# anrieff/fray

Measured on AMD Instinct MI355X. Metric: Mrays/s (closest-hit + shadow rays) at 1920x1080, 64spp path trace, higher is better.
Workload: dtype f64

## Files before the change

fray_amd/csrc/adaptive_variant.hip:

```cpp
#include "adaptive.hpp"
#include "dev_compact.hpp"
#include "render_impl.hpp"

#ifndef FRAY_ST
#error "compile with -DFRAY_ST=0..5, 8 or 9"
#endif

namespace {

struct ListBatch {
    const int* list;
    int p0, np, s0, cn;
};

static __global__ __launch_bounds__(256) void k_seed_list(DFrame F, ListBatch B, uint32_t* __restrict__ x397)
{
    constexpr int NC = FRAY_SEED_CHAINS;
    const uint32_t total = (uint32_t)B.np * (uint32_t)B.cn;
    const uint32_t groups = (total + NC - 1u) / NC;
    for (uint32_t q = blockIdx.x * blockDim.x + threadIdx.x; q < groups; q += gridDim.x * blockDim.x) {
        uint32_t b[NC], slot[NC];
#pragma unroll
        for (int k = 0; k < NC; k++) {
            slot[k] = q + (uint32_t)k * groups;
// ... 25 lines not shown
        const int i = (int)(slot % (uint32_t)B.np), s = (int)(slot / (uint32_t)B.np);
        int x, y;
        item_pixel(F, B.list[B.p0 + i], x, y);
        PathState ps;
        const uint32_t p = (uint32_t)y * (uint32_t)F.W + (uint32_t)x;
        ps.rnd = mt_seed_with(sample_seed(F.seed, p, (uint32_t)(B.s0 + s)), x397[slot]);
        ps.tab = ps.rnd;
        float ox = rng_float(ps.rnd), oy = rng_float(ps.rnd);
        double fx = (double)((float)x + ox), fy = (double)((float)y + oy);
        if (C.dof) dof_ray(C, fx, fy, ps.tab, ps.o, ps.d); else screen_ray(C, fx, fy, ps.o, ps.d);
        ps.pm = c3(1, 1, 1);
        ps.slot = slot;
        ps.depth = 0;
        ps.flags = 0;
        c.samples++;
        path_store<FRAY_SORT && sort_variant(ST)>(Q, slot, ps, ray_sort_class<ST>(ps.d, 0u));
        termCount[slot] = 0;
    }
    if (ST & 1) flush_stats(st, c);
    else if (c.samples) atomicAdd(&st->samples, c.samples);
}

struct PixelState {
    float* sum;
    float* prev;
    unsigned char* flag;
};

struct ResolveArgs {
    DFrame F;
    ListBatch B;
// ... 218 lines not shown
```

fray_amd/csrc/capi.hip:

```cpp
#include <hip/hip_runtime.h>

#include <algorithm>
#include <chrono>
#include <cstddef>
#include <cmath>
#include <cstring>
#include <string>
#include <vector>
#include <functional>
#include <cstdlib>


#include "entry_support.hpp"
#include "dev_rng.hpp"
#include "dev_pack.hpp"
#include "scene_arena.hpp"

namespace {

using frayhip_detail::set_error;

void put3(double* o, const double* p) { o[0] = p[0]; o[1] = p[1]; o[2] = p[2]; }
}

// ... 215 lines not shown
    if (s->settings.gi) spp = std::max(spp, s->settings.numPaths);
    return spp;
}

DScene frame_scene(const frayhip_scene* s)
{
    const frayhip_settings& set = s->settings;
    DScene S = s->S;
    S.ambient[0] = set.ambientLight[0]; S.ambient[1] = set.ambientLight[1]; S.ambient[2] = set.ambientLight[2];
    S.maxTraceDepth = set.maxTraceDepth;
    S.gi = set.gi;
    S.saturation = set.saturation;
    S.skipNullSegments = s->skipNullSegments ? 1 : 0;
    S.segmentPlanes = s->segmentPlanes ? 1 : 0;
    S.certifiedSegments = (s->certifiedSegments && s->segmentPlanes && S.segCertAll) ? 1 : 0;
    if (!s->cameraSkip) S.nCamSkip = 0;
    if (!s->shadeShortcuts) S.shadeIdentity = S.lightsDiagonal = S.subdShift = 0;
    return S;
}

DFrame frame_record(const frayhip_scene* s, int bucketFirst, int bucketStride, uint32_t seed)
{
    DFrame F = frame_grid(s->settings.frameWidth, s->settings.frameHeight);
    F.bucketStride = bucketStride > 0 ? bucketStride : 1;
    F.bucketFirst = bucketFirst;
    F.nBuckets = frayhip_bucket_count(F.W, F.H, F.bucketFirst, F.bucketStride);
    F.spp = frame_spp(s);
    F.seed = seed;
    F.jitter = (s->camera.dof || s->settings.gi) ? 1 : 0;
    return F;
// ... 305 lines not shown
    sc->edit = make_scene_edit(d, B);
    sc->camera = d.camera;
    sc->settings = d.settings;
    if (hipMalloc((void**)&sc->d_stats, kStatsBytes) != hipSuccess || hipMalloc((void**)&sc->d_qmeta, 3 * FRAY_PT_LANES * sizeof(QMeta)) != hipSuccess ||
        hipEventCreate(&sc->evA) != hipSuccess || hipEventCreate(&sc->evB) != hipSuccess || !create_lanes(sc)) {
        set_error("frayhip_scene_create: could not allocate the per-scene device state");
        frayhip_scene_destroy(sc);
        return FRAYHIP_E_NOMEM;
    }
    if (const char* e = getenv("FRAYHIP_PT_LANES")) { long v = atol(e); if (v >= 1 && v <= FRAY_PT_LANES) sc->ptLanes = (int)v; }
    if (const char* e = getenv("FRAYHIP_SPECULATE_FANS")) sc->speculateFans = atol(e) != 0;
    if (const char* e = getenv("FRAYHIP_FP_CONTRACT")) sc->fpContract = atol(e) == 1;
    if (const char* e = getenv("FRAYHIP_SKIP_NULL_SEGMENTS")) sc->skipNullSegments = atol(e) != 0;
    if (const char* e = getenv("FRAYHIP_SEGMENT_PLANES")) sc->segmentPlanes = atol(e) != 0;
    if (const char* e = getenv("FRAYHIP_CERTIFIED_SEGMENTS")) sc->certifiedSegments = atol(e) != 0;
    if (const char* e = getenv("FRAYHIP_TIGHT_GATES")) sc->tightGates = atol(e) != 0;
    if (const char* e = getenv("FRAYHIP_CAMERA_SKIP")) sc->cameraSkip = atol(e) != 0;
    if (const char* e = getenv("FRAYHIP_CAMERA_TILES")) sc->cameraTiles = atol(e) != 0;
    if (const char* e = getenv("FRAYHIP_SHADE_SHORTCUTS")) sc->shadeShortcuts = atol(e) != 0;
    if (const char* e = getenv("FRAYHIP_FUSED_WHITTED_MAX")) { long v = atol(e); if (v >= 0 && v <= 1024) sc->fusedWhittedMax = (int)v; }
    if (const char* e = getenv("FRAYHIP_CSG_LANES")) { long v = atol(e); if (v >= 1 && v <= FRAY_PT_LANES) sc->csgLanes = (int)v; }
    if (const char* e = getenv("FRAYHIP_SEED_TABLE_MIB")) { long v = atol(e); if (v >= 0 && v <= (1 << 20)) sc->seedTableCapBytes = (size_t)v << 20; }
    if (const char* e = getenv("FRAYHIP_PT_BUDGET_MIB")) { long v = atol(e); if (v >= 1 && v <= (1 << 20)) { sc->ptBudgetBytes = (size_t)v << 20; sc->ptBudgetEff = 0; } }
    *out = sc;
    return FRAYHIP_OK;
}

int frayhip_scene_get_option(frayhip_scene* s, const char* name, int64_t* value)
{
    if (!s || !name || !value) { set_error("frayhip_scene_get_option: null argument"); return FRAYHIP_E_ARG; }
// ... 355 lines not shown
```

fray_amd/csrc/dev_scene.hpp:

```cpp
#pragma once
#include <stdint.h>
#include "frayhip.h"
#include "dev_tricert.hpp"
#include "dev_segcert.hpp"
#include "dev_gatecert.hpp"

#ifdef __HIP_DEVICE_COMPILE__
#define FRAY_RO __attribute__((address_space(4)))
#else
#define FRAY_RO
#endif

#define FRAY_CSG_MAX 30
#ifndef FRAY_CSG_DEPTH
#define FRAY_CSG_DEPTH 16
#endif

#define FRAY_KD_LDS_STACK 16
#define FRAY_KD_MAX_DEPTH 72

struct DXform { double off[3]; double m[9]; double inv[9]; };

struct DTri;
struct DNode {
// ... 126 lines not shown
    const FRAY_RO DLight* lights;
    DEnv env;
    int32_t nNodes, nLights;
    float probPickLight;
    float ambient[3];
    int32_t maxTraceDepth, gi;
    float saturation;
    const FRAY_RO DSegPlane* segPlanes;
    const FRAY_RO uint32_t* segNodeMasks;
    int32_t nSegPlanes, nSegNodes;
    int32_t segmentPlanes;
    int32_t skipNullSegments;
    int32_t segCertAll;
    int32_t certifiedSegments;
    const FRAY_RO DCamSkip* camSkip;
    int32_t nCamSkip, padCamSkip;
    const FRAY_RO double* worldNormals;
    int32_t normStride, shadeIdentity, lightsDiagonal;
    int32_t subdShift;
};

struct DFrame {
    int32_t W, H, BW, BH;
    int32_t bucketFirst, bucketStride, nBuckets , spp;
    uint32_t seed;
    int32_t jitter;
};

struct DStats {
    unsigned long long closest, shadow, node, kdInner, leafRefs, tri, prim, smooth, samples, tex, rngOverflow;
#ifdef FRAY_STAMPS
// ... 6 lines not shown
```

fray_amd/csrc/kernels.hpp:

```cpp
#pragma once
#include "dev_shade.hpp"
#include "dev_whitted.hpp"
#include "dev_queues.hpp"
#include "dev_camtile.hpp"
#include <type_traits>

#ifndef FRAY_PRIMARY_WAVES
#define FRAY_PRIMARY_WAVES 5
#endif
#ifndef FRAY_WHITTED_WAVES
#define FRAY_WHITTED_WAVES 3
#endif
#ifndef FRAY_WHITTED_REFILL
#define FRAY_WHITTED_REFILL 64
#endif
#ifndef FRAY_CSG_WAVES
#define FRAY_CSG_WAVES 3
#endif
constexpr int waves_for(int st, int n) { return (st & 2) ? (FRAY_CSG_WAVES < n ? FRAY_CSG_WAVES : n) : ((st & 1) && n > 2 ? n - 1 : n); }
#ifndef FRAY_MT_EARLY
#define FRAY_MT_EARLY 160
#endif
#ifndef FRAY_WH_SHADE_WAVES
#define FRAY_WH_SHADE_WAVES 4
// ... 748 lines not shown

#ifndef FRAY_SORT
#define FRAY_SORT 1
#endif
#ifndef FRAY_SORT_N
#define FRAY_SORT_N 1024
#endif
#ifdef FRAY_SORT_BY_MATERIAL
constexpr bool sort_variant(int) { return true; }
#else
#ifndef FRAY_SORT_CSG
#define FRAY_SORT_CSG 0
#endif
constexpr bool sort_variant(int st) { return (st & 6) == 4 || (FRAY_SORT_CSG && (st & 2) != 0); }
#endif
FD void wave_lds_sync()
{
    __builtin_amdgcn_fence(__ATOMIC_RELEASE, "wavefront");
    __builtin_amdgcn_wave_barrier();
    __builtin_amdgcn_fence(__ATOMIC_ACQUIRE, "wavefront");
}
template <class KeyOf>
FD void sort_share(const FRAY_RO uint32_t* off, const FRAY_RO uint32_t* nf, uint32_t nSeg, uint32_t chunk, uint32_t b0, uint32_t b1, uint32_t& seg,
                   uint32_t* buf, uint32_t* cnt, KeyOf keyOf)
{
    const uint32_t lane = threadIdx.x & 63u;
    if (lane < 16) cnt[lane] = 0;
    wave_lds_sync();
    uint32_t s1 = seg;
    for (uint32_t base = b0; base < b1; base += 64u) {
        const uint32_t di = base + lane;
        const bool live = di < b1;
        const uint32_t i = seg_map(off, nf, nSeg, chunk, base, di, live, s1) & ~FRAY_FRONT_BIT;
        if (live) atomicAdd(cnt + keyOf(i), 1u);
    }
    wave_lds_sync();
    {
        const uint32_t v = lane < 16 ? cnt[lane] : 0u;
        uint32_t inc = v;
        for (int d = 1; d < 16; d <<= 1) { const uint32_t t = __shfl_up(inc, d, 64); if ((int)lane >= d) inc += t; }
        wave_lds_sync();
        if (lane < 16) cnt[lane] = inc - v;
    }
    wave_lds_sync();
    uint32_t s2 = seg;
    for (uint32_t base = b0; base < b1; base += 64u) {
        const uint32_t di = base + lane;
        const bool live = di < b1;
        const uint32_t raw = seg_map(off, nf, nSeg, chunk, base, di, live, s2);
        if (live) buf[atomicAdd(cnt + keyOf(raw & ~FRAY_FRONT_BIT), 1u)] = raw;
    }
    seg = s2;
    wave_lds_sync();
}

template <class G>
FD void path_finish(const TermBuf& TB, DStats* st, const PathStateT<G>& s, const StereoBuf& SB)
{
    const Mt &r = cursor(s.rnd), &t = cursor(s.tab);
    if (SB.g[0]) {
        SB.g[0][s.slot] = r.j; SB.g[1][s.slot] = r.a; SB.g[2][s.slot] = r.b;
        SB.g[3][s.slot] = t.j; SB.g[4][s.slot] = t.a; SB.g[5][s.slot] = t.b;
    }
    TB.n[s.slot] = (unsigned short)(TB.b + 1);
    if (sizeof(G) == sizeof(Mt) && (r.j > 227 || t.j > 227)) atomicAdd(&st->rngOverflow, 1ull);
}
FD void term_store(const TermBuf& TB, uint32_t slot, C3 v)
// ... 28 lines not shown
                    if (C.dof) dof_ray(C, fx, fy, ps.tab, ro, rd, 2); else screen_ray(C, fx, fy, ro, rd, 2);
                    SB.r[0][slot] = ro.x; SB.r[1][slot] = ro.y; SB.r[2][slot] = ro.z;
                    SB.r[3][slot] = rd.x; SB.r[4][slot] = rd.y; SB.r[5][slot] = rd.z;
                }
            } else {
                ps.rnd.j = SB.g[0][slot]; ps.rnd.a = SB.g[1][slot]; ps.rnd.b = SB.g[2][slot];
                ps.tab.j = SB.g[3][slot]; ps.tab.a = SB.g[4][slot]; ps.tab.b = SB.g[5][slot];
                ps.o = v3(SB.r[0][slot], SB.r[1][slot], SB.r[2][slot]);
                ps.d = v3(SB.r[3][slot], SB.r[4][slot], SB.r[5][slot]);
            }
            ps.pm = c3(1, 1, 1);
            ps.slot = slot;
            ps.depth = 0;
            ps.flags = 0;
            bump<ST>(c.samples);
            path_store<FRAY_SORT && sort_variant(ST)>(Q, slot, ps, ray_sort_class<ST>(ps.d, 0u));
        } else {
            PathRec* r = Q.rec + slot;
            r->d[0] = 0; r->d[1] = 0; r->d[2] = 0;
            r->depthFlags = FRAY_DEAD;
            if constexpr (FRAY_SORT && sort_variant(ST)) Q.cls[slot] = 15;
        }
        termCount[slot] = 0;
    }
    if (ST & 1) flush_stats(st, c);
}

struct WaveShare { uint32_t begin, end, chunk, w, W; };
FD WaveShare wave_share(uint32_t n)
{
    WaveShare r;
    r.W = gridDim.x * (blockDim.x >> 6);
    r.w = blockIdx.x * (blockDim.x >> 6) + (threadIdx.x >> 6);
    r.chunk = (((n + r.W - 1u) / r.W) + 63u) & ~63u;
    r.begin = r.w * r.chunk;
    r.end = r.begin + r.chunk < n ? r.begin + r.chunk : n;
// ... 49 lines not shown
                if constexpr (ST == 0 && FRAY_ARITH == 0) { if (S.certifiedSegments) planesPass = segment_certified(S, sa, sb); }
                shadowBack = ray_gate_class<tight_variant(ST)>(S, sa, sb - sa);
                if constexpr (ST == 0) {
                    if (FRAY_ARITH == 0 ? planesPass && shadowBack == 0 : segment_surely_visible(S, sa, sb, shadowBack)) {
                        own = sc;
                        shadow = false;
                        atomicAdd(shadowEnds.n + 2, 1u);
                    }
                }
                if (ST != 0 || shadow) {
                    const uint32_t j = seg_take(shadowEnds, shadowBack != 0);
                    SQ.ax[j] = sa.x; SQ.ay[j] = sa.y; SQ.az[j] = sa.z;
                    SQ.bx[j] = sb.x; SQ.by[j] = sb.y; SQ.bz[j] = sb.z;
                    SQ.cr[j] = sc.r; SQ.cg[j] = sc.g; SQ.cb[j] = sc.b;
                    SQ.slot[j] = ps.slot;
                    if constexpr (FRAY_SORT && sort_variant(ST)) SQ.cls[j] = (unsigned char)ray_sort_class<ST>(sb - sa, shadowBack);
                }
            }
        }
        PathRay win, wout;
        win.o = ps.o; win.d = ps.d; win.depth = ps.depth; win.flags = ps.flags;
        C3 brdf;
        float pdf;
        spawn_ray(sh, info, win, ps.tab, wout, brdf, pdf);
        {
            ps.pm = ps.pm * brdf / pdf;
            ps.o = wout.o; ps.d = wout.d; ps.depth = wout.depth; ps.flags = wout.flags;
#ifdef FRAY_SORT_BY_MATERIAL
            ps.flags = (ps.flags & 0xffu) | ((sh.kind == 1 ? 0u : sh.kind == 3 ? 1u : sh.kind == 4 ? 2u : 3u) << 8);
#endif
            if (ps.depth > S.maxTraceDepth || intensity(ps.pm) < 0.01) path_finish(TB, st, ps, SB);
// ... 20 lines not shown
        const CamTileRays R = cam_tile_rays(V, x0, y0);
        for (int r = 0; r < A.nRecs; r++) {
            if (!tile_surely_misses_box(A.recs[r], V, R)) continue;
            if (tile_surely_guarded(A.recs[r], R)) skip |= 1u << A.recs[r].node; else ask |= 1u << A.recs[r].node;
        }
    }
    DCamTile e;
    e.skip = skip; e.x0 = (uint16_t)x0; e.y0 = (uint16_t)y0;
    A.out[t] = e;
    A.ask[t] = ask;
}

#ifndef FRAY_ARITH
#define FRAY_ARITH 0
#endif
template <int ST, bool LONG, bool FIRST = false, int ARITH = FRAY_ARITH>
static __global__ __launch_bounds__(256, waves_for(ST, kd_variant(ST) ? FRAY_BOUNCE_WAVES : FRAY_BOUNCE_WAVES_NOKD)) void k_pt_bounce(BounceArgs A)
{
    static_assert(!(LONG && FIRST), "long generators start from k_pt_init");
    typedef typename std::conditional<LONG, MtPath, Mt>::type G;
    Cnt c = zero_cnt();
    const QMetaRO metaIn = A.metaIn;
    QMeta* const metaOut = A.metaOut;
    QMeta* const metaShadow = A.metaShadow;
    DStats* const st = A.st;
    const FRAY_RO uint32_t* off = FIRST ? nullptr : metaIn.p->off;
    const FRAY_RO uint32_t* nfIn = FIRST ? nullptr : metaIn.p->nf;
    const uint32_t nSeg = FIRST ? 1u : metaIn.p->nSeg, chunkIn = FIRST ? A.FA.n : metaIn.p->chunk;
    const bool certFront = !FIRST && metaIn.p->certFront != 0;
    const WaveShare ws = wave_share(FIRST ? A.FA.n : metaIn.p->n);
    const uint32_t lane = threadIdx.x & 63u;
    SegEnds outEnds{ws.begin, ws.chunk, 0, 0};
    __shared__ uint32_t shadowCount[4][ST == 0 ? 3 : 2];
    if (lane < (ST == 0 ? 3u : 2u)) shadowCount[threadIdx.x >> 6][lane] = 0;
    const SegEndsShared shadowEnds{ws.begin, ws.chunk, shadowCount[threadIdx.x >> 6]};
    uint32_t seg = (!FIRST && ws.begin < ws.end) ? seg_first(off, nSeg, ws.begin) : 0;
#ifdef FRAY_STAMPS
    stamp_begin();
#endif
    constexpr bool CAMSKIP = FIRST && tight_variant(ST);
    uint32_t camSkipped = 0, camWaves = 0;
    constexpr bool SORT = FRAY_SORT && !FIRST && sort_variant(ST);
    const uint32_t sortN = (uint32_t)FRAY_SORT_N;
    for (uint32_t b0 = ws.begin, b1 = 0; b0 < ws.end; b0 = b1) {
    b1 = (SORT && ws.end - b0 > sortN) ? b0 + sortN : ws.end;
    uint32_t* sorted = nullptr;
    if constexpr (SORT) {
        __shared__ uint32_t sortBuf[4][FRAY_SORT_N];
        __shared__ uint32_t sortCnt[4][16];
        sorted = sortBuf[threadIdx.x >> 6];
        const unsigned char* const cls = KARG(BounceArgs, kernel_args<BounceArgs>(), Qin).cls;
        sort_share(off, nfIn, nSeg, chunkIn, b0, b1, seg, sorted, sortCnt[threadIdx.x >> 6], [&](uint32_t i) { return (uint32_t)cls[i] & 15u; });
    }
    for (uint32_t base = b0; base < b1; base += 64u) {
        const FRAY_RO BounceArgs* AP = kernel_args<BounceArgs>();
        const FirstArgs& FA = KARG(BounceArgs, AP, FA);
        const DScene& S = KARG(BounceArgs, AP, S);
        const PathQueue& Qin = KARG(BounceArgs, AP, Qin);
        const PathQueue& Qout = KARG(BounceArgs, AP, Qout);
        const ShadowQueue& SQ = KARG(BounceArgs, AP, SQ);
        const TermBuf& TB = KARG(BounceArgs, AP, TB);
        const StereoBuf& SB = KARG(BounceArgs, AP, SB);
        const LongRng& LR = KARG(BounceArgs, AP, LR);
        const uint32_t di = base + lane;
        bool cont = false, shadow = false, gateFree = false;
        uint32_t shadowBack = 0;
        PathStateT<G> ps;
// ... 78 lines not shown
                ps.rnd.seed = ps.tab.seed = sd;
                ps.rnd.stride = ps.tab.stride = LR.nPaths;
                ps.rnd.col = LR.cols + ps.slot;
                ps.tab.col = LR.cols + (size_t)624 * LR.nPaths + ps.slot;
            }
            STAMP(8);
            path_shade<ST, false>(S, ps, h, TB, st, SB, cont, shadow, shadowBack, SQ, shadowEnds, c);
            STAMP(10);
        }
        const uint32_t gate = cont ? ray_gate_class<tight_variant(ST)>(S, ps.o, ps.d) : 0u;
        const bool back = gate != 0;
        const uint32_t slotOut = seg_slot(outEnds, cont, back);
#ifdef FRAY_SORT_BY_MATERIAL
        if (cont) path_store<true>(Qout, slotOut, ps, (ps.flags >> 8) & 3u);
#else
        if (cont) path_store<FRAY_SORT && sort_variant(ST)>(Qout, slotOut, ps, ray_sort_class<ST>(ps.d, gate));
#endif
        seg_advance(outEnds, cont, back);
        STAMP(13);
    }
    }
#ifdef FRAY_STAMPS
    if (lane < 24) { atomicAdd(&st->stamp[lane], g_stampAcc[threadIdx.x >> 6][lane]); atomicAdd(&st->stampLanes[lane], g_stampLanes[threadIdx.x >> 6][lane]); }
#endif
    if (lane == 0) {
        metaOut->cnt[ws.w] = outEnds.nF + outEnds.nB; metaOut->nf[ws.w] = outEnds.nF;
        metaShadow->cnt[ws.w] = shadowCount[threadIdx.x >> 6][0] + shadowCount[threadIdx.x >> 6][1]; metaShadow->nf[ws.w] = shadowCount[threadIdx.x >> 6][0];
        if constexpr (ST == 0) {
            unsigned long long* const total = KARG(BounceArgs, kernel_args<BounceArgs>(), segCertified);
            const uint32_t nCert = shadowCount[threadIdx.x >> 6][2];
            if (total && nCert) atomicAdd(total, (unsigned long long)nCert);
        }
        if constexpr (CAMSKIP) {
            unsigned long long* const pairs = KARG(BounceArgs, kernel_args<BounceArgs>(), camSkipped);
            if (pairs && camWaves) { atomicAdd(pairs, (unsigned long long)camSkipped); atomicAdd(pairs + 1, (unsigned long long)camWaves); }
        }
    }
    if (blockIdx.x == 0 && threadIdx.x == 0) {
        metaOut->chunk = ws.chunk; metaOut->nSeg = ws.W; metaShadow->chunk = ws.chunk; metaShadow->nSeg = ws.W;
        metaOut->certFront = metaShadow->certFront = A.S.gatesExact ? 1u : 0u;
    }
    if (ST & 1) flush_stats(st, c);
    if ((ST & 2) && c.envelope) atomicAdd(&st->rngOverflow, 1ull);
}

struct ShadowArgs { DScene S; ShadowQueue SQ; QMetaRO meta; TermBuf TB; DStats* st; unsigned long long* segSkipped; };
template <int ST, int ARITH = FRAY_ARITH>
static __global__ __launch_bounds__(256, anyhit_waves(ST)) void k_pt_shadow(ShadowArgs A)
{
    Cnt c = zero_cnt();
    const QMetaRO meta = A.meta;
    DStats* const st = A.st;
    const FRAY_RO uint32_t* off = meta.p->off;
    const FRAY_RO uint32_t* nfIn = meta.p->nf;
    const uint32_t nSeg = meta.p->nSeg, chunkIn = meta.p->chunk;
    const bool certFront = meta.p->certFront != 0;
    const WaveShare ws = wave_share(meta.p->n);
    const uint32_t lane = threadIdx.x & 63u;
    if (ws.begin >= ws.end) return;
    uint32_t seg = seg_first(off, nSeg, ws.begin);
#ifdef FRAY_STAMPS
    stamp_begin();
#endif
    constexpr bool SORT = FRAY_SORT && sort_variant(ST);
    constexpr bool SEGP = identity_variant(ST) && !(ST & 1);
    uint32_t segSkipped = 0;
    const uint32_t sortN = (uint32_t)FRAY_SORT_N;
    for (uint32_t b0 = ws.begin, b1 = 0; b0 < ws.end; b0 = b1) {
    b1 = (SORT && ws.end - b0 > sortN) ? b0 + sortN : ws.end;
    uint32_t* sorted = nullptr;
    if constexpr (SORT) {
        __shared__ uint32_t sortBuf[4][FRAY_SORT_N];
        __shared__ uint32_t sortCnt[4][16];
        sorted = sortBuf[threadIdx.x >> 6];
        const unsigned char* const cls = KARG(ShadowArgs, kernel_args<ShadowArgs>(), SQ).cls;
        sort_share(off, nfIn, nSeg, chunkIn, b0, b1, seg, sorted, sortCnt[threadIdx.x >> 6], [&](uint32_t i) { return (uint32_t)cls[i] & 15u; });
    }
    for (uint32_t base = b0; base < b1; base += 64u) {
        const FRAY_RO ShadowArgs* AP = kernel_args<ShadowArgs>();
        const DScene& S = KARG(ShadowArgs, AP, S);
        const ShadowQueue& SQ = KARG(ShadowArgs, AP, SQ);
        const TermBuf& TB = KARG(ShadowArgs, AP, TB);
        const uint32_t di = base + lane;
        const bool live = di < b1;
        uint32_t i;
        if constexpr (SORT) i = live ? sorted[di - b0] : 0u;
        else i = seg_map(off, nfIn, nSeg, chunkIn, base, di, live, seg);
        const bool gateFree = certFront && (i & FRAY_FRONT_BIT);
        i &= ~FRAY_FRONT_BIT;
        if constexpr (SEGP) {
            V3 a = v3(0, 0, 0), b = a;
// ... 144 lines not shown
```

fray_amd/csrc/render_contract.hip:

```cpp
#ifndef FRAY_ARITH
#error "compile with -DFRAY_ARITH=1 -ffp-contract=fast"
#endif
#include "render_state.hpp"
#include "kernels.hpp"

#ifndef FRAY_ST
#error "compile with -DFRAY_ST=0..5, 8 or 9"
#endif

namespace frayhip_detail {
template <int ST> void launch_bounce_contracted(int grid, hipStream_t stream, const BounceArgs& A)
{
    hipLaunchKernelGGL((k_pt_bounce<ST, false, false, FRAY_ARITH>), dim3(grid), dim3(256), 0, stream, A);
}
template <int ST> void launch_shadow_contracted(int grid, hipStream_t stream, const ShadowArgs& A)
{
    hipLaunchKernelGGL((k_pt_shadow<ST, FRAY_ARITH>), dim3(grid), dim3(256), 0, stream, A);
}
template void launch_bounce_contracted<FRAY_ST>(int, hipStream_t, const BounceArgs&);
template void launch_shadow_contracted<FRAY_ST>(int, hipStream_t, const ShadowArgs&);
}

#if FRAY_ST == 0
static __global__ __launch_bounds__(256) void k_debug_arith(int op, int n, const double* __restrict__ a, const double* __restrict__ b, double* __restrict__ out)
{
#ifdef __HIP_DEVICE_COMPILE__
    for (int i = blockIdx.x * blockDim.x + threadIdx.x; i < n; i += gridDim.x * blockDim.x) {
        switch (op) {
// ... 39 lines not shown
```

fray_amd/csrc/render_impl.hpp:

```cpp
#pragma once
#include <algorithm>
#include <chrono>
#include <cstring>
#include <cstdio>

#include "accum.hpp"
#include "entry_support.hpp"
#include "kernels.hpp"

namespace frayhip_detail {

namespace {
unsigned char* carve_queue(unsigned char* p, size_t n, PathQueue& Q)
{
    Carve c{p};
    Q.rec = (PathRec*)c.take(n * sizeof(PathRec));
    Q.cls = c.take(n);
    return c.p;
}
size_t queue_bytes(size_t n) { return r256(n * sizeof(PathRec)) + r256(n); }
unsigned char* carve_shadow(unsigned char* p, size_t n, ShadowQueue& Q)
{
    Carve c{p};
    Q.ax = (double*)c.take(n * 8); Q.ay = (double*)c.take(n * 8); Q.az = (double*)c.take(n * 8);
// ... 6 lines not shown
size_t shadow_bytes(size_t n) { return 6 * r256(n * 8) + 4 * r256(n * 4) + r256(n); }

template <int ST>
int pt_bounces(frayhip_scene* sc, const DScene& S, const PathQueue (&Q)[2], const ShadowQueue& SQ, TermBuf TB, int nBounce, int grid, hipStream_t stream,
               size_t& nTraceEvents, size_t& nShadowEvents)
{
    QMeta* meta = sc->d_qmeta;
    for (int b = 0; b < nBounce; b++) {
        const QMetaRO mIn{(const FRAY_RO QMeta*)(meta + (b & 1))}, mSh{(const FRAY_RO QMeta*)(meta + 2)};
        hipEvent_t ea = pool_event(sc->evPool, nTraceEvents), eb = pool_event(sc->evPool, nTraceEvents + 1);
        hipEvent_t ec = pool_event(sc->evPoolShadow, nShadowEvents), ed = pool_event(sc->evPoolShadow, nShadowEvents + 1);
        if (!ea || !eb || !ec || !ed) return FRAYHIP_E_NOMEM;
        TB.b = b;
        const BounceArgs BA{S, Q[b & 1], Q[(b + 1) & 1], SQ, mIn, meta + ((b + 1) & 1), meta + 2, TB, StereoBuf{}, LongRng{}, sc->d_stats, FirstArgs{}};
        HIP_TRY(hipEventRecord(ea, stream));
        hipLaunchKernelGGL((k_pt_bounce<ST, false>), dim3(grid), dim3(256), 0, stream, BA);
        HIP_TRY(hipEventRecord(eb, stream));
        nTraceEvents += 2;
        hipLaunchKernelGGL(k_scan, dim3(2), dim3(1024), 0, stream, meta + ((b + 1) & 1), meta + 2, (unsigned long long*)nullptr);
        HIP_TRY(hipEventRecord(ec, stream));
        hipLaunchKernelGGL(k_pt_shadow<ST>, dim3(grid), dim3(256), 0, stream, ShadowArgs{S, SQ, mSh, TB, sc->d_stats + 1, (unsigned long long*)((unsigned char*)sc->d_stats + kSegSkippedOffset)});
        HIP_TRY(hipEventRecord(ed, stream));
        nShadowEvents += 2;
    }
    return FRAYHIP_OK;
}

inline int seed_batch(frayhip_scene* sc, const DFrame& F, int nItems, int s0, int cn, uint32_t* scratch, hipStream_t ls, const uint32_t*& out)
{
    auto launch = [&](int a, int n, uint32_t* to) {
        hipLaunchKernelGGL(k_seed, dim3(seed_grid(((size_t)nItems * n + FRAY_SEED_CHAINS - 1) / FRAY_SEED_CHAINS)), dim3(256), 0, ls, F, nItems, a, n, to);
// ... 346 lines not shown
            if (ST & 2) maxLanes = std::max(1, std::min(maxLanes, sc->csgLanes));
            if (ST & 1) maxLanes = 1;
            const bool longRngW = long_generators(set.maxTraceDepth);
            const unsigned warmKey = 1u << ((longRngW ? 1 : 0) | (sc->fpContract ? 2 : 0) | (sc->camera.stereoSeparation > 0 ? 4 : 0));
            if (maxLanes > 1 && !(sc->warmMask & warmKey) && !getenv("FRAYHIP_NO_PRIME")) {
                HIP_TRY(hipMemsetAsync(sc->d_qmeta, 0, 3 * FRAY_PT_LANES * sizeof(QMeta), stream));
                HIP_TRY(hipStreamSynchronize(stream));
                for (int k = 0; k < maxLanes; k++) {
                    hipStream_t ws = k == 0 ? stream : sc->laneStream[k];
                    QMeta* m = sc->d_qmeta + 3 * k;
                    const QMetaRO mIn{(const FRAY_RO QMeta*)m};
                    BounceArgs BA{};
                    BA.S = S; BA.metaIn = mIn; BA.metaOut = m + 1; BA.metaShadow = m + 2; BA.st = sc->d_stats;
                    ShadowArgs SA{};
                    SA.S = S; SA.meta = mIn; SA.st = sc->d_stats + 1;
                    if (longRngW) hipLaunchKernelGGL((k_pt_bounce<ST, true>), dim3(1), dim3(256), 0, ws, BA);
                    else {
                        hipLaunchKernelGGL((k_pt_bounce<ST, false>), dim3(1), dim3(256), 0, ws, BA);
                        hipLaunchKernelGGL((k_pt_bounce<ST, false, true>), dim3(1), dim3(256), 0, ws, BA);
                    }
                    hipLaunchKernelGGL(k_pt_shadow<ST>, dim3(1), dim3(256), 0, ws, SA);
                    if constexpr (!(ST & 2)) {
                        if (sc->fpContract) { launch_bounce_contracted<ST>(1, ws, BA); launch_shadow_contracted<ST>(1, ws, SA); }
                    }
                    HIP_TRY(hipStreamSynchronize(ws));
                }
                sc->warmMask |= warmKey;
            }
            if (maxLanes > 3 && (size_t)nItems * (size_t)spp < ((size_t)24 << 20)) maxLanes = 3;
            const bool stereo = sc->camera.stereoSeparation > 0;
            int chunk = 0, nBatches = 0, nLanes = 0;
            size_t nPaths = 0, nQueue = 0, laneBytes = 0;
            if (first == 0) seed_table_begin(sc, F, nItems, spp);
            for (;;) {
// ... 96 lines not shown
                        if (!ea || !eb || !ec || !ed) return FRAYHIP_E_NOMEM;
                        HIP_TRY(hipEventRecord(ea, ls));
                        const LongRng LR{L.mtCols, (uint32_t)nPaths, F, nItems, s0};
                        const TermBuf TB{L.terms, L.termCount, (uint32_t)nPaths, b};
                        const FirstArgs FA{C, F, nItems, s0, (uint32_t)((size_t)nItems * cn), x397, L.termCount, (const FRAY_RO DCamTile*)tiles, (const FRAY_RO uint32_t*)(tiles ? tileAsk : nullptr)};
                        const BounceArgs BA{S, L.Q[b & 1], L.Q[(b + 1) & 1], L.SQ, mIn, L.meta + ((b + 1) & 1), L.meta + 2, TB, save, LR, sc->d_stats, FA, L.segCertified, L.camSkipped};
                        bool contractedLaunch = false;
                        if constexpr (!(ST & 2)) {
                            if (sc->fpContract && !longRng && b > 0) {
                                BounceArgs BC = BA;
                                BC.S.gates = sc->S.gates;
                                launch_bounce_contracted<ST>(grid, ls, BC); contractedLaunch = true; nContracted++;
                            }
                        }
                        if (contractedLaunch) {}
                        else if (longRng) hipLaunchKernelGGL((k_pt_bounce<ST, true>), dim3(grid), dim3(256), 0, ls, BA);
                        else if (fused && b == 0) hipLaunchKernelGGL((k_pt_bounce<ST, false, true>), dim3(grid), dim3(256), 0, ls, BA);
                        else hipLaunchKernelGGL((k_pt_bounce<ST, false>), dim3(grid), dim3(256), 0, ls, BA);
                        HIP_TRY(hipEventRecord(eb, ls));
                        nTraceEvents += 2;
                        hipLaunchKernelGGL(k_scan, dim3(2), dim3(1024), 0, ls, L.meta + ((b + 1) & 1), L.meta + 2, L.segTotal);
                        HIP_TRY(hipEventRecord(ec, ls));
                        bool contractedShadow = false;
                        if constexpr (!(ST & 2)) {
                            if (sc->fpContract) { launch_shadow_contracted<ST>(grid, ls, ShadowArgs{S, L.SQ, mSh, TB, sc->d_stats + 1, L.segSkipped}); contractedShadow = true; nContracted++; }
                        }
                        if (!contractedShadow) hipLaunchKernelGGL(k_pt_shadow<ST>, dim3(grid), dim3(256), 0, ls, ShadowArgs{S, L.SQ, mSh, TB, sc->d_stats + 1, L.segSkipped});
                        HIP_TRY(hipEventRecord(ed, ls));
                        nShadowEvents += 2;
                    }
                    if (stereo) hipLaunchKernelGGL(k_pt_fold, dim3(grid_for((size_t)nItems * cn)), dim3(256), 0, ls, TermBuf{L.terms, L.termCount, (uint32_t)nPaths, 0},
                                                   (uint32_t)((size_t)nItems * cn), rad);
                }
// ... 112 lines not shown
```

fray_amd/csrc/render_state.hpp:

```cpp
#pragma once
#include <hip/hip_runtime.h>

#include <cstddef>
#include <string>
#include <vector>

#include "capi_common.h"
#include "dev_scene.hpp"
#include "dev_queues.hpp"

namespace frayhip_detail {
inline int hip_error_code(hipError_t e)
{
    switch (e) {
        case hipErrorOutOfMemory: return FRAYHIP_E_NOMEM;
        case hipErrorNoDevice: case hipErrorInvalidDevice: case hipErrorInsufficientDriver: case hipErrorNotInitialized: return FRAYHIP_E_NODEVICE;
        default: return FRAYHIP_E_HIP;
    }
}
}
#define HIP_TRY(expr)                                                                             \
    do {                                                                                          \
        hipError_t e_ = (expr);                                                                   \
        if (e_ != hipSuccess) {                                                                   \
// ... 39 lines not shown
    bool speculateFans = true;
    bool lightDraws = false;
    int lastWhittedPath = 0;
    int fusedWhittedMax = 4;
    int csgLanes = 1;
    unsigned warmMask = 0;
    bool fpContract = false;
    long long lastContracted = 0;
    bool skipNullSegments = true;
    bool segmentPlanes = true;
    bool certifiedSegments = true;
    bool tightGates = true;
    bool cameraSkip = true;
    bool shadeShortcuts = true;
    bool cameraTiles = true;
    long long lastCameraSkipped = 0, lastCameraWaves = 0;
    long long lastShadowCertified = 0;
    long long lastShadowNodesSkipped = 0;
    long long lastShadowSegments = 0;
    long long lastFans[4] = {0, 0, 0, 0};
    int lightSampleCount = 0;
    bool extGeometry = false;
    bool textured = false;
    bool kdMeshes = false;
    void* d_work = nullptr;
    size_t work_bytes = 0;
    DStats* d_stats = nullptr;
    void* d_motionTab = nullptr;
    size_t motionTabBytes = 0;
    std::vector<unsigned char> motionTabHost;
// ... 45 lines not shown
```

fray_amd/csrc/samplemap_variant.hip:

```cpp
#include "samplemap.hpp"
#include "dev_compact.hpp"
#include "render_impl.hpp"

#ifndef FRAY_ST
#error "compile with -DFRAY_ST=0..5, 8 or 9"
#endif

namespace {

struct MapHead {
    int count;
    int slots;
    int bad;
    int addMax;
    int cntMaxInv, cntMax;
    unsigned long long samples;
    unsigned long long pixels;
};

struct MapBatch {
    const int* list;
    int p0, np, k0, cn;
    const int32_t* add;
    const int32_t* count;
// ... 147 lines not shown
        int x, y;
        uint32_t s;
        map_slot(F, B, slot, x, y, s);
        PathState ps;
        const uint32_t p = (uint32_t)y * (uint32_t)F.W + (uint32_t)x;
        ps.rnd = mt_seed_with(sample_seed(F.seed, p, s), x397[slot]);
        ps.tab = ps.rnd;
        float ox = rng_float(ps.rnd), oy = rng_float(ps.rnd);
        double fx = (double)((float)x + ox), fy = (double)((float)y + oy);
        if (C.dof) dof_ray(C, fx, fy, ps.tab, ps.o, ps.d); else screen_ray(C, fx, fy, ps.o, ps.d);
        ps.pm = c3(1, 1, 1);
        ps.slot = slot;
        ps.depth = 0;
        ps.flags = 0;
        c.samples++;
        path_store<FRAY_SORT && sort_variant(ST)>(Q, slot, ps, ray_sort_class<ST>(ps.d, 0u));
        termCount[slot] = 0;
    }
    if (ST & 1) flush_stats(st, c);
    else if (c.samples) atomicAdd(&st->samples, c.samples);
}

FD float map_lum(C3 c) { return ((c.r + c.g) + c.b) / 3.0f; }
FD void map_add(float4& row, C3 c)
{
    const C3 a = c3(row.x, row.y, row.z) + c;
    const float l = map_lum(c);
    row.x = a.r; row.y = a.g; row.z = a.b;
    row.w = row.w + l * l;
}

// ... 401 lines not shown
```

fray_amd/csrc/scene_arena.hpp:

```cpp
#pragma once
#include <algorithm>
#include <cmath>
#include <cstddef>
#include <cstdint>
#include <cstring>
#include <functional>
#include <vector>

#include "dev_scene.hpp"

namespace frayhip_arena {

struct ArenaTable { uint64_t off, bytes; };

struct ArenaMeshTables { int32_t tris, attrs, kd, kdBox, refs, ltris, ltris32; };

struct ArenaFacts {
    int32_t extGeometry, kdMeshes, textured, whittedNeedsRecursion, lightDraws, lightSampleCount, specFanMax;
    int32_t nGates, gatesExact, nSegPlanes, nSegNodes, segCertAll;
    int32_t nTightGates;
    int32_t nCamSkip, tCamSkip;
    int32_t shadeIdentity, lightsDiagonal;
    int32_t normStride, tWorldNormals;
    int32_t nNodes, nLights, nMeshes, nTextures;
// ... 586 lines not shown
    }
    DNode* const nodes = (DNode*)write[F.tNodes];
    for (int i = 0; i < F.nNodes; i++)
        if (nodes[i].geomKind == FRAYHIP_GEOM_MESH && !meshes[nodes[i].geomIndex].hasKd) nodes[i].tlPtr = meshes[nodes[i].geomIndex].tris;
    DTexture* const tex = (DTexture*)write[F.tTex];
    for (int i = 0; i < F.nTextures; i++) tex[i].texels = (const FRAY_RO float*)addr[F.tTexels] + texelOffset[i];

    S.nodes = (const FRAY_RO DNode*)addr[F.tNodes];
    S.nodesX = (const FRAY_RO DNodeX*)addr[F.tNodesX];
    S.gates = (const FRAY_RO DGate*)addr[F.tGates];
    S.nGates = F.nGates; S.gatesExact = F.gatesExact;
    S.segPlanes = (const FRAY_RO DSegPlane*)addr[F.tSegPlanes];
    S.segNodeMasks = (const FRAY_RO uint32_t*)addr[F.tSegMasks];
    S.nSegPlanes = F.nSegPlanes; S.nSegNodes = F.nSegNodes; S.segCertAll = F.segCertAll;
    S.camSkip = (const FRAY_RO DCamSkip*)addr[F.tCamSkip];
    S.nCamSkip = F.nCamSkip; S.padCamSkip = 0;
    S.worldNormals = (const FRAY_RO double*)addr[F.tWorldNormals];
    S.normStride = F.normStride; S.shadeIdentity = F.shadeIdentity; S.lightsDiagonal = F.lightsDiagonal; S.subdShift = 1;
    S.planes = (const FRAY_RO DPlane*)addr[F.tPlanes];
    S.spheres = (const FRAY_RO DSphere*)addr[F.tSpheres];
    S.cubes = (const FRAY_RO DCube*)addr[F.tCubes];
    S.csgs = (const FRAY_RO DCsg*)addr[F.tCsgs];
    S.meshes = (const FRAY_RO DMesh*)addr[F.tMeshes];
    S.shaders = (const FRAY_RO DShader*)addr[F.tShaders];
    S.layers = (const FRAY_RO DLayer*)addr[F.tLayers];
    S.textures = (const FRAY_RO DTexture*)addr[F.tTex];
    S.lights = (const FRAY_RO DLight*)addr[F.tLights];
    S.env.present = F.envPresent;
    S.env.loaded = F.envLoaded;
    for (int f = 0; f < 6; f++) {
        S.env.width[f] = F.envWidth[f];
// ... 10 lines not shown
```

fray_amd/csrc/shade_variant.hip:

```cpp
#include "shade.hpp"
#include "render_impl.hpp"

#ifndef FRAY_ST
#error "compile with -DFRAY_ST=0..5, 8 or 9"
#endif

namespace {

struct ShadeRays {
    const double* org;
    const double* dir;
    const uint32_t* keys;
    uint32_t seed;
    int r0, nr, s0, cn, skip;
};

FD bool finite3(V3 v) { return fabs(v.x) <= __DBL_MAX__ && fabs(v.y) <= __DBL_MAX__ && fabs(v.z) <= __DBL_MAX__; }
FD bool load_ray(const ShadeRays& R, int g, V3& o, V3& d)
{
    const double* po = R.org + 3 * (size_t)g;
    const double* pd = R.dir + 3 * (size_t)g;
    o = v3(po[0], po[1], po[2]);
    d = v3(pd[0], pd[1], pd[2]);
    const double dd = d.x * d.x + d.y * d.y + d.z * d.z;
// ... 116 lines not shown
{
    Cnt c = zero_cnt();
    const uint32_t total = (uint32_t)R.nr * (uint32_t)R.cn;
    for (uint32_t slot = blockIdx.x * blockDim.x + threadIdx.x; slot < total; slot += gridDim.x * blockDim.x) {
        const int k = (int)(slot / (uint32_t)R.nr), g = R.r0 + (int)(slot - (uint32_t)k * (uint32_t)R.nr);
        PathState ps;
        if (load_ray(R, g, ps.o, ps.d)) {
            ps.rnd = mt_seed_with(sample_seed(R.seed, ray_key(R, g), (uint32_t)(R.s0 + k)), x397[slot]);
            ps.tab = ps.rnd;
            mt_skip(ps.rnd, R.skip);
            ps.pm = c3(1, 1, 1);
            ps.slot = slot;
            ps.depth = 0;
            ps.flags = 0;
            c.samples++;
            path_store<FRAY_SORT && sort_variant(ST)>(Q, slot, ps, ray_sort_class<ST>(ps.d, 0u));
        } else {
            PathRec* r = Q.rec + slot;
            r->d[0] = 0; r->d[1] = 0; r->d[2] = 0;
            r->depthFlags = FRAY_DEAD;
            if constexpr (FRAY_SORT && sort_variant(ST)) Q.cls[slot] = 15;
        }
        termCount[slot] = 0;
    }
    flush_query<ST>(st, c);
}

static __global__ __launch_bounds__(256) void k_shade_resolve(int nr, int s, int cn, int spp, const float* __restrict__ rad, float* __restrict__ sum, float* __restrict__ rgb)
{
    for (int i = blockIdx.x * blockDim.x + threadIdx.x; i < nr; i += gridDim.x * blockDim.x) {
        const size_t si = (size_t)i * 3;
        C3 a = s == 0 ? c3(0, 0, 0) : c3(sum[si], sum[si + 1], sum[si + 2]);
        for (int k = 0; k < cn; k++) {
            const size_t q = ((size_t)k * nr + i) * 3;
            a = a + c3(rad[q], rad[q + 1], rad[q + 2]);
        }
// ... 148 lines not shown
```

include/frayhip.h:

```cpp
#ifndef FRAYHIP_H
#define FRAYHIP_H

#include <stdint.h>

#ifdef __cplusplus
extern "C" {
#endif

#define FRAYHIP_ABI_VERSION 3

enum {
    FRAYHIP_OK            = 0,
    FRAYHIP_E_ARG         = -1,
    FRAYHIP_E_PARSE       = -2,
    FRAYHIP_E_NODEVICE    = -3,
    FRAYHIP_E_UNSUPPORTED = -4,
    FRAYHIP_E_NOMEM       = -5,
    FRAYHIP_E_HIP         = -6,
    FRAYHIP_E_CANCELLED   = -7,
};


typedef struct frayhip_transform {
    double offset[3];
// ... 185 lines not shown
int  frayhip_scene_update(frayhip_scene* s, const frayhip_scene_desc* desc);

int  frayhip_transform_identity(frayhip_transform* T);
int  frayhip_transform_scale(frayhip_transform* T, double x, double y, double z);
int  frayhip_transform_rotate(frayhip_transform* T, double yaw, double pitch, double roll);
int  frayhip_transform_translate(frayhip_transform* T, double x, double y, double z);
int  frayhip_light_begin_frame(frayhip_light* light);
int  frayhip_shader_begin_frame(frayhip_shader* shader);

int  frayhip_scene_set_option(frayhip_scene* s, const char* name, int64_t value);
int  frayhip_scene_get_option(frayhip_scene* s, const char* name, int64_t* value);
int  frayhip_scene_tight_gates(frayhip_scene* s, int enable, int64_t* enabled, int64_t* eligible);
int  frayhip_scene_camera_skip(frayhip_scene* s, int enable, int64_t* enabled, int64_t* eligible, int64_t* skipped, int64_t* waves);
int  frayhip_scene_camera_tiles(frayhip_scene* s, int enable, int64_t* enabled);
int  frayhip_scene_shade_shortcuts(frayhip_scene* s, int enable, int64_t* enabled, int64_t* eligible);

int  frayhip_render(frayhip_scene* s, const frayhip_frame* f,
                    float* rgb, int32_t* hit_id, double* hit_dist, frayhip_stats* st);
int  frayhip_render_device(frayhip_scene* s, const frayhip_frame* f,
                           float* d_rgb, int32_t* d_hit_id, double* d_hit_dist,
                           void* hip_stream, frayhip_stats* st);

typedef struct frayhip_progress {
    int32_t samples_done;
    int32_t samples_total;
    int32_t batches_done, batches_total;
    double  ms_elapsed;
    int32_t preview;
    int32_t final;
    const float* rgb;
// ... 299 lines not shown
```

Baseline: 14300.

## Rewrite wave sort with ballot ranking and add opt-in sorted bounce kernel

The per-wave counting sort used before bounce and shadow tracing now keeps the window's keys in registers and ranks them with ballot/mbcnt instead of two passes of LDS atomics, removing the second seg_map walk. It also stamps sort classes on path records in identity variants and adds a second bounce kernel that sorts rays by direction class, chosen at launch by a new sortBounces flag (env FRAYHIP_SORT_BOUNCES, off by default). The register-held window raises register pressure, and the extra class stamping adds stores in identity variants even when bounce sorting is off.

```diff
diff --git a/fray_amd/csrc/adaptive_variant.hip b/fray_amd/csrc/adaptive_variant.hip
--- a/fray_amd/csrc/adaptive_variant.hip
+++ b/fray_amd/csrc/adaptive_variant.hip
@@ -63,7 +63,7 @@
         ps.depth = 0;
         ps.flags = 0;
         c.samples++;
-        path_store<FRAY_SORT && sort_variant(ST)>(Q, slot, ps, ray_sort_class<ST>(ps.d, 0u));
+        path_store<FRAY_SORT && sort_path_variant(ST)>(Q, slot, ps, ray_sort_class<ST>(ps.d, 0u));
         termCount[slot] = 0;
     }
     if (ST & 1) flush_stats(st, c);
diff --git a/fray_amd/csrc/capi.hip b/fray_amd/csrc/capi.hip
--- a/fray_amd/csrc/capi.hip
+++ b/fray_amd/csrc/capi.hip
@@ -253,6 +253,7 @@
     S.skipNullSegments = s->skipNullSegments ? 1 : 0;
     S.segmentPlanes = s->segmentPlanes ? 1 : 0;
     S.certifiedSegments = (s->certifiedSegments && s->segmentPlanes && S.segCertAll) ? 1 : 0;
+    S.sortBounces = s->sortBounces ? 1 : 0;
     if (!s->cameraSkip) S.nCamSkip = 0;
     if (!s->shadeShortcuts) S.shadeIdentity = S.lightsDiagonal = S.subdShift = 0;
     return S;
@@ -588,6 +589,7 @@
     if (const char* e = getenv("FRAYHIP_SKIP_NULL_SEGMENTS")) sc->skipNullSegments = atol(e) != 0;
     if (const char* e = getenv("FRAYHIP_SEGMENT_PLANES")) sc->segmentPlanes = atol(e) != 0;
     if (const char* e = getenv("FRAYHIP_CERTIFIED_SEGMENTS")) sc->certifiedSegments = atol(e) != 0;
+    if (const char* e = getenv("FRAYHIP_SORT_BOUNCES")) sc->sortBounces = atol(e) != 0;
     if (const char* e = getenv("FRAYHIP_TIGHT_GATES")) sc->tightGates = atol(e) != 0;
     if (const char* e = getenv("FRAYHIP_CAMERA_SKIP")) sc->cameraSkip = atol(e) != 0;
     if (const char* e = getenv("FRAYHIP_CAMERA_TILES")) sc->cameraTiles = atol(e) != 0;
diff --git a/fray_amd/csrc/dev_scene.hpp b/fray_amd/csrc/dev_scene.hpp
--- a/fray_amd/csrc/dev_scene.hpp
+++ b/fray_amd/csrc/dev_scene.hpp
@@ -164,7 +164,8 @@
     int32_t segCertAll;
     int32_t certifiedSegments;
     const FRAY_RO DCamSkip* camSkip;
-    int32_t nCamSkip, padCamSkip;
+    int32_t nCamSkip;
+    int32_t sortBounces;
     const FRAY_RO double* worldNormals;
     int32_t normStride, shadeIdentity, lightsDiagonal;
     int32_t subdShift;
diff --git a/fray_amd/csrc/kernels.hpp b/fray_amd/csrc/kernels.hpp
--- a/fray_amd/csrc/kernels.hpp
+++ b/fray_amd/csrc/kernels.hpp
@@ -786,6 +786,9 @@
 #endif
 constexpr bool sort_variant(int st) { return (st & 6) == 4 || (FRAY_SORT_CSG && (st & 2) != 0); }
 #endif
+constexpr bool sort_shadow_variant(int st) { return sort_variant(st); }
+constexpr bool sort_switch_variant(int st) { return FRAY_SORT && !sort_variant(st) && identity_variant(st); }
+constexpr bool sort_path_variant(int st) { return sort_variant(st) || sort_switch_variant(st); }
 FD void wave_lds_sync()
 {
     __builtin_amdgcn_fence(__ATOMIC_RELEASE, "wavefront");
@@ -794,35 +797,56 @@
 }
 template <class KeyOf>
 FD void sort_share(const FRAY_RO uint32_t* off, const FRAY_RO uint32_t* nf, uint32_t nSeg, uint32_t chunk, uint32_t b0, uint32_t b1, uint32_t& seg,
-                   uint32_t* buf, uint32_t* cnt, KeyOf keyOf)
-{
+                   uint32_t* buf, KeyOf keyOf)
+{
+    constexpr int NG = FRAY_SORT_N / 64;
+    static_assert(FRAY_SORT_N % 64 == 0 && NG >= 1 && NG <= 32, "a window is whole wave-loads, each lane holding one entry of each in a register");
     const uint32_t lane = threadIdx.x & 63u;
-    if (lane < 16) cnt[lane] = 0;
+    uint32_t raw[NG], key[NG];
+    uint32_t s = seg;
+#pragma unroll
+    for (int g = 0; g < NG; g++) {
+        const uint32_t base = b0 + 64u * (uint32_t)g;
+        raw[g] = 0; key[g] = 16u;
+        if (base < b1) {
+            const bool live = base + lane < b1;
+            raw[g] = seg_map(off, nf, nSeg, chunk, base, base + lane, live, s);
+            if (live) key[g] = keyOf(raw[g] & ~FRAY_FRONT_BIT);
+        }
+    }
+    seg = s;
+    uint32_t run[16];
+#pragma unroll
+    for (int c = 0; c < 16; c++) run[c] = 0;
+#pragma unroll
+    for (int g = 0; g < NG; g++) {
+        if (b0 + 64u * (uint32_t)g < b1) {
+            uint32_t r = 0;
+#pragma unroll
+            for (int c = 0; c < 16; c++) {
+                const unsigned long long m = __ballot(key[g] == (uint32_t)c);
+                const uint32_t mine = __builtin_amdgcn_mbcnt_hi((uint32_t)(m >> 32), __builtin_amdgcn_mbcnt_lo((uint32_t)m, run[c]));
+                if (key[g] == (uint32_t)c) r = mine;
+                run[c] += (uint32_t)__popcll(m);
+            }
+            key[g] |= r << 8;
+        }
+    }
+    uint32_t tot = 0;
+#pragma unroll
+    for (int c = 0; c < 16; c++) tot = lane == (uint32_t)c ? run[c] : tot;
+    uint32_t inc = tot;
+    for (int d = 1; d < 16; d <<= 1) { const uint32_t t = __shfl_up(inc, d, 64); if ((int)lane >= d) inc += t; }
+    const uint32_t first = inc - tot;
     wave_lds_sync();
-    uint32_t s1 = seg;
-    for (uint32_t base = b0; base < b1; base += 64u) {
-        const uint32_t di = base + lane;
-        const bool live = di < b1;
-        const uint32_t i = seg_map(off, nf, nSeg, chunk, base, di, live, s1) & ~FRAY_FRONT_BIT;
-        if (live) atomicAdd(cnt + keyOf(i), 1u);
-    }
-    wave_lds_sync();
-    {
-        const uint32_t v = lane < 16 ? cnt[lane] : 0u;
-        uint32_t inc = v;
-        for (int d = 1; d < 16; d <<= 1) { const uint32_t t = __shfl_up(inc, d, 64); if ((int)lane >= d) inc += t; }
-        wave_lds_sync();
-        if (lane < 16) cnt[lane] = inc - v;
-    }
-    wave_lds_sync();
-    uint32_t s2 = seg;
-    for (uint32_t base = b0; base < b1; base += 64u) {
-        const uint32_t di = base + lane;
-        const bool live = di < b1;
-        const uint32_t raw = seg_map(off, nf, nSeg, chunk, base, di, live, s2);
-        if (live) buf[atomicAdd(cnt + keyOf(raw & ~FRAY_FRONT_BIT), 1u)] = raw;
-    }
-    seg = s2;
+#pragma unroll
+    for (int g = 0; g < NG; g++) {
+        if (b0 + 64u * (uint32_t)g < b1) {
+            const uint32_t k = key[g] & 255u;
+            const uint32_t at = (uint32_t)__shfl((int)first, (int)(k & 15u), 64) + (key[g] >> 8);
+            if (k < 16u) buf[at] = raw[g];
+        }
+    }
     wave_lds_sync();
 }
 
@@ -881,12 +905,12 @@
             ps.depth = 0;
             ps.flags = 0;
             bump<ST>(c.samples);
-            path_store<FRAY_SORT && sort_variant(ST)>(Q, slot, ps, ray_sort_class<ST>(ps.d, 0u));
+            path_store<FRAY_SORT && sort_path_variant(ST)>(Q, slot, ps, ray_sort_class<ST>(ps.d, 0u));
         } else {
             PathRec* r = Q.rec + slot;
             r->d[0] = 0; r->d[1] = 0; r->d[2] = 0;
             r->depthFlags = FRAY_DEAD;
-            if constexpr (FRAY_SORT && sort_variant(ST)) Q.cls[slot] = 15;
+            if constexpr (FRAY_SORT && sort_path_variant(ST)) Q.cls[slot] = 15;
         }
         termCount[slot] = 0;
     }
@@ -966,7 +990,7 @@
                     SQ.bx[j] = sb.x; SQ.by[j] = sb.y; SQ.bz[j] = sb.z;
                     SQ.cr[j] = sc.r; SQ.cg[j] = sc.g; SQ.cb[j] = sc.b;
                     SQ.slot[j] = ps.slot;
-                    if constexpr (FRAY_SORT && sort_variant(ST)) SQ.cls[j] = (unsigned char)ray_sort_class<ST>(sb - sa, shadowBack);
+                    if constexpr (FRAY_SORT && sort_shadow_variant(ST)) SQ.cls[j] = (unsigned char)ray_sort_class<ST>(sb - sa, shadowBack);
                 }
             }
         }
@@ -1017,10 +1041,11 @@
 #ifndef FRAY_ARITH
 #define FRAY_ARITH 0
 #endif
-template <int ST, bool LONG, bool FIRST = false, int ARITH = FRAY_ARITH>
-static __global__ __launch_bounds__(256, waves_for(ST, kd_variant(ST) ? FRAY_BOUNCE_WAVES : FRAY_BOUNCE_WAVES_NOKD)) void k_pt_bounce(BounceArgs A)
+template <int ST, bool LONG, bool FIRST, bool SORTED>
+FD void pt_bounce(const BounceArgs& A)
 {
     static_assert(!(LONG && FIRST), "long generators start from k_pt_init");
+    static_assert(!SORTED || sort_switch_variant(ST), "the variants that always sort, and those that never do, have no second kernel");
     typedef typename std::conditional<LONG, MtPath, Mt>::type G;
     Cnt c = zero_cnt();
     const QMetaRO metaIn = A.metaIn;
@@ -1043,17 +1068,17 @@
 #endif
     constexpr bool CAMSKIP = FIRST && tight_variant(ST);
     uint32_t camSkipped = 0, camWaves = 0;
-    constexpr bool SORT = FRAY_SORT && !FIRST && sort_variant(ST);
+    constexpr bool STAMP_CLS = FRAY_SORT && (sort_variant(ST) || SORTED);
+    constexpr bool SORT = STAMP_CLS && !FIRST;
     const uint32_t sortN = (uint32_t)FRAY_SORT_N;
     for (uint32_t b0 = ws.begin, b1 = 0; b0 < ws.end; b0 = b1) {
     b1 = (SORT && ws.end - b0 > sortN) ? b0 + sortN : ws.end;
     uint32_t* sorted = nullptr;
     if constexpr (SORT) {
         __shared__ uint32_t sortBuf[4][FRAY_SORT_N];
-        __shared__ uint32_t sortCnt[4][16];
         sorted = sortBuf[threadIdx.x >> 6];
         const unsigned char* const cls = KARG(BounceArgs, kernel_args<BounceArgs>(), Qin).cls;
-        sort_share(off, nfIn, nSeg, chunkIn, b0, b1, seg, sorted, sortCnt[threadIdx.x >> 6], [&](uint32_t i) { return (uint32_t)cls[i] & 15u; });
+        sort_share(off, nfIn, nSeg, chunkIn, b0, b1, seg, sorted, [&](uint32_t i) { return (uint32_t)cls[i] & 15u; });
     }
     for (uint32_t base = b0; base < b1; base += 64u) {
         const FRAY_RO BounceArgs* AP = kernel_args<BounceArgs>();
@@ -1162,7 +1187,7 @@
 #ifdef FRAY_SORT_BY_MATERIAL
         if (cont) path_store<true>(Qout, slotOut, ps, (ps.flags >> 8) & 3u);
 #else
-        if (cont) path_store<FRAY_SORT && sort_variant(ST)>(Qout, slotOut, ps, ray_sort_class<ST>(ps.d, gate));
+        if (cont) path_store<STAMP_CLS>(Qout, slotOut, ps, ray_sort_class<ST>(ps.d, gate));
 #endif
         seg_advance(outEnds, cont, back);
         STAMP(13);
@@ -1190,6 +1215,24 @@
     }
     if (ST & 1) flush_stats(st, c);
     if ((ST & 2) && c.envelope) atomicAdd(&st->rngOverflow, 1ull);
+}
+template <int ST, bool LONG, bool FIRST = false, int ARITH = FRAY_ARITH>
+static __global__ __launch_bounds__(256, waves_for(ST, kd_variant(ST) ? FRAY_BOUNCE_WAVES : FRAY_BOUNCE_WAVES_NOKD)) void k_pt_bounce(BounceArgs A)
+{
+    pt_bounce<ST, LONG, FIRST, false>(A);
+}
+template <int ST, bool LONG, bool FIRST = false, int ARITH = FRAY_ARITH>
+static __global__ __launch_bounds__(256, waves_for(ST, kd_variant(ST) ? FRAY_BOUNCE_WAVES : FRAY_BOUNCE_WAVES_NOKD)) void k_pt_bounce_sorted(BounceArgs A)
+{
+    pt_bounce<ST, LONG, FIRST, true>(A);
+}
+template <int ST, bool LONG, bool FIRST = false>
+static void launch_bounce(int grid, hipStream_t stream, const BounceArgs& A)
+{
+    if constexpr (sort_switch_variant(ST)) {
+        if (A.S.sortBounces) { hipLaunchKernelGGL((k_pt_bounce_sorted<ST, LONG, FIRST>), dim3(grid), dim3(256), 0, stream, A); return; }
+    }
+    hipLaunchKernelGGL((k_pt_bounce<ST, LONG, FIRST>), dim3(grid), dim3(256), 0, stream, A);
 }
 
 struct ShadowArgs { DScene S; ShadowQueue SQ; QMetaRO meta; TermBuf TB; DStats* st; unsigned long long* segSkipped; };
@@ -1210,7 +1253,7 @@
 #ifdef FRAY_STAMPS
     stamp_begin();
 #endif
-    constexpr bool SORT = FRAY_SORT && sort_variant(ST);
+    constexpr bool SORT = FRAY_SORT && sort_shadow_variant(ST);
     constexpr bool SEGP = identity_variant(ST) && !(ST & 1);
     uint32_t segSkipped = 0;
     const uint32_t sortN = (uint32_t)FRAY_SORT_N;
@@ -1219,10 +1262,9 @@
     uint32_t* sorted = nullptr;
     if constexpr (SORT) {
         __shared__ uint32_t sortBuf[4][FRAY_SORT_N];
-        __shared__ uint32_t sortCnt[4][16];
         sorted = sortBuf[threadIdx.x >> 6];
         const unsigned char* const cls = KARG(ShadowArgs, kernel_args<ShadowArgs>(), SQ).cls;
-        sort_share(off, nfIn, nSeg, chunkIn, b0, b1, seg, sorted, sortCnt[threadIdx.x >> 6], [&](uint32_t i) { return (uint32_t)cls[i] & 15u; });
+        sort_share(off, nfIn, nSeg, chunkIn, b0, b1, seg, sorted, [&](uint32_t i) { return (uint32_t)cls[i] & 15u; });
     }
     for (uint32_t base = b0; base < b1; base += 64u) {
         const FRAY_RO ShadowArgs* AP = kernel_args<ShadowArgs>();
diff --git a/fray_amd/csrc/render_contract.hip b/fray_amd/csrc/render_contract.hip
--- a/fray_amd/csrc/render_contract.hip
+++ b/fray_amd/csrc/render_contract.hip
@@ -11,7 +11,7 @@
 namespace frayhip_detail {
 template <int ST> void launch_bounce_contracted(int grid, hipStream_t stream, const BounceArgs& A)
 {
-    hipLaunchKernelGGL((k_pt_bounce<ST, false, false, FRAY_ARITH>), dim3(grid), dim3(256), 0, stream, A);
+    launch_bounce<ST, false>(grid, stream, A);
 }
 template <int ST> void launch_shadow_contracted(int grid, hipStream_t stream, const ShadowArgs& A)
 {
diff --git a/fray_amd/csrc/render_impl.hpp b/fray_amd/csrc/render_impl.hpp
--- a/fray_amd/csrc/render_impl.hpp
+++ b/fray_amd/csrc/render_impl.hpp
@@ -44,7 +44,7 @@
         TB.b = b;
         const BounceArgs BA{S, Q[b & 1], Q[(b + 1) & 1], SQ, mIn, meta + ((b + 1) & 1), meta + 2, TB, StereoBuf{}, LongRng{}, sc->d_stats, FirstArgs{}};
         HIP_TRY(hipEventRecord(ea, stream));
-        hipLaunchKernelGGL((k_pt_bounce<ST, false>), dim3(grid), dim3(256), 0, stream, BA);
+        launch_bounce<ST, false>(grid, stream, BA);
         HIP_TRY(hipEventRecord(eb, stream));
         nTraceEvents += 2;
         hipLaunchKernelGGL(k_scan, dim3(2), dim3(1024), 0, stream, meta + ((b + 1) & 1), meta + 2, (unsigned long long*)nullptr);
@@ -421,10 +421,10 @@
                     BA.S = S; BA.metaIn = mIn; BA.metaOut = m + 1; BA.metaShadow = m + 2; BA.st = sc->d_stats;
                     ShadowArgs SA{};
                     SA.S = S; SA.meta = mIn; SA.st = sc->d_stats + 1;
-                    if (longRngW) hipLaunchKernelGGL((k_pt_bounce<ST, true>), dim3(1), dim3(256), 0, ws, BA);
+                    if (longRngW) launch_bounce<ST, true>(1, ws, BA);
                     else {
-                        hipLaunchKernelGGL((k_pt_bounce<ST, false>), dim3(1), dim3(256), 0, ws, BA);
-                        hipLaunchKernelGGL((k_pt_bounce<ST, false, true>), dim3(1), dim3(256), 0, ws, BA);
+                        launch_bounce<ST, false>(1, ws, BA);
+                        launch_bounce<ST, false, true>(1, ws, BA);
                     }
                     hipLaunchKernelGGL(k_pt_shadow<ST>, dim3(1), dim3(256), 0, ws, SA);
                     if constexpr (!(ST & 2)) {
@@ -551,9 +551,9 @@
                             }
                         }
                         if (contractedLaunch) {}
-                        else if (longRng) hipLaunchKernelGGL((k_pt_bounce<ST, true>), dim3(grid), dim3(256), 0, ls, BA);
-                        else if (fused && b == 0) hipLaunchKernelGGL((k_pt_bounce<ST, false, true>), dim3(grid), dim3(256), 0, ls, BA);
-                        else hipLaunchKernelGGL((k_pt_bounce<ST, false>), dim3(grid), dim3(256), 0, ls, BA);
+                        else if (longRng) launch_bounce<ST, true>(grid, ls, BA);
+                        else if (fused && b == 0) launch_bounce<ST, false, true>(grid, ls, BA);
+                        else launch_bounce<ST, false>(grid, ls, BA);
                         HIP_TRY(hipEventRecord(eb, ls));
                         nTraceEvents += 2;
                         hipLaunchKernelGGL(k_scan, dim3(2), dim3(1024), 0, ls, L.meta + ((b + 1) & 1), L.meta + 2, L.segTotal);
diff --git a/fray_amd/csrc/render_state.hpp b/fray_amd/csrc/render_state.hpp
--- a/fray_amd/csrc/render_state.hpp
+++ b/fray_amd/csrc/render_state.hpp
@@ -77,6 +77,7 @@
     bool cameraSkip = true;
     bool shadeShortcuts = true;
     bool cameraTiles = true;
+    bool sortBounces = false;
     long long lastCameraSkipped = 0, lastCameraWaves = 0;
     long long lastShadowCertified = 0;
     long long lastShadowNodesSkipped = 0;
diff --git a/fray_amd/csrc/samplemap_variant.hip b/fray_amd/csrc/samplemap_variant.hip
--- a/fray_amd/csrc/samplemap_variant.hip
+++ b/fray_amd/csrc/samplemap_variant.hip
@@ -185,7 +185,7 @@
         ps.depth = 0;
         ps.flags = 0;
         c.samples++;
-        path_store<FRAY_SORT && sort_variant(ST)>(Q, slot, ps, ray_sort_class<ST>(ps.d, 0u));
+        path_store<FRAY_SORT && sort_path_variant(ST)>(Q, slot, ps, ray_sort_class<ST>(ps.d, 0u));
         termCount[slot] = 0;
     }
     if (ST & 1) flush_stats(st, c);
diff --git a/fray_amd/csrc/scene_arena.hpp b/fray_amd/csrc/scene_arena.hpp
--- a/fray_amd/csrc/scene_arena.hpp
+++ b/fray_amd/csrc/scene_arena.hpp
@@ -624,7 +624,7 @@
     S.segNodeMasks = (const FRAY_RO uint32_t*)addr[F.tSegMasks];
     S.nSegPlanes = F.nSegPlanes; S.nSegNodes = F.nSegNodes; S.segCertAll = F.segCertAll;
     S.camSkip = (const FRAY_RO DCamSkip*)addr[F.tCamSkip];
-    S.nCamSkip = F.nCamSkip; S.padCamSkip = 0;
+    S.nCamSkip = F.nCamSkip; S.sortBounces = 0;
     S.worldNormals = (const FRAY_RO double*)addr[F.tWorldNormals];
     S.normStride = F.normStride; S.shadeIdentity = F.shadeIdentity; S.lightsDiagonal = F.lightsDiagonal; S.subdShift = 1;
     S.planes = (const FRAY_RO DPlane*)addr[F.tPlanes];
diff --git a/fray_amd/csrc/shade_variant.hip b/fray_amd/csrc/shade_variant.hip
--- a/fray_amd/csrc/shade_variant.hip
+++ b/fray_amd/csrc/shade_variant.hip
@@ -154,12 +154,12 @@
             ps.depth = 0;
             ps.flags = 0;
             c.samples++;
-            path_store<FRAY_SORT && sort_variant(ST)>(Q, slot, ps, ray_sort_class<ST>(ps.d, 0u));
+            path_store<FRAY_SORT && sort_path_variant(ST)>(Q, slot, ps, ray_sort_class<ST>(ps.d, 0u));
         } else {
             PathRec* r = Q.rec + slot;
             r->d[0] = 0; r->d[1] = 0; r->d[2] = 0;
             r->depthFlags = FRAY_DEAD;
-            if constexpr (FRAY_SORT && sort_variant(ST)) Q.cls[slot] = 15;
+            if constexpr (FRAY_SORT && sort_path_variant(ST)) Q.cls[slot] = 15;
         }
         termCount[slot] = 0;
     }
diff --git a/include/frayhip.h b/include/frayhip.h
--- a/include/frayhip.h
+++ b/include/frayhip.h
@@ -223,6 +223,7 @@
 int  frayhip_scene_camera_skip(frayhip_scene* s, int enable, int64_t* enabled, int64_t* eligible, int64_t* skipped, int64_t* waves);
 int  frayhip_scene_camera_tiles(frayhip_scene* s, int enable, int64_t* enabled);
 int  frayhip_scene_shade_shortcuts(frayhip_scene* s, int enable, int64_t* enabled, int64_t* eligible);
+
 
 int  frayhip_render(frayhip_scene* s, const frayhip_frame* f,
                     float* rgb, int32_t* hit_id, double* hit_dist, frayhip_stats* st);
```

Result: no change. 14250 (-0.3%).
